# simochen/flowtrack.pytorch

Measured on AMD Instinct MI355X. Metric: pose crops/sec (ResNet-50 + 3-deconv head, 256x192), higher is better.
Workload: dtype fp16; 1 GPU; ResNet-50 pose head fp16, batch 64 x 256x192 synthetic crops per GPU (BASELINE.json configs[1]); per_gpu_batch=64, resident_batches=4, parallelism=dp1: batch sharded, one process per GPU

## Files before the change

### flowtrack/pytorch_amd/build.py

```python
from __future__ import annotations

import hashlib
import os
import subprocess
import sys

HERE = os.path.dirname(os.path.abspath(__file__))
ROOT = os.path.dirname(os.path.dirname(HERE))
CSRC = os.path.join(HERE, "csrc")
INCLUDE = os.path.join(ROOT, "include")
LIB_PATH = os.path.join(HERE, "libflowtrack_hip.so")
STAMP_PATH = os.path.join(HERE, ".libflowtrack_hip.stamp")

SOURCES = ["conv_igemm.hip", "conv_igemm8.hip", "bottleneck.hip", "bottleneck_rstat.hip", "bottleneck_stream.hip", "bottleneck_cluster.hip", "conv_direct.hip", "conv_wstat.hip", "aux_ops.hip", "flow_ops.hip", "crop_ops.hip", "runtime.hip"]
HEADERS = [os.path.join(CSRC, "ft_common.h"), os.path.join(CSRC, "conv_common.h"), os.path.join(CSRC, "conv_wstat.h"), os.path.join(INCLUDE, "flowtrack_hip.h")]
EXPORTS = os.path.join(CSRC, "exports.map")
ARCH = "gfx950"
FLAGS = ["-O3", "-std=c++17", "-fPIC", "-Wall", "-Wno-unused-function"]


def _hipcc() -> str:
    for cand in (os.environ.get("HIPCC"), "/opt/rocm/bin/hipcc", "hipcc"):
        if cand and (os.path.isabs(cand) and os.path.exists(cand) or not os.path.isabs(cand)):
            return cand
    raise RuntimeError("hipcc not found")


def _fingerprint() -> str:
    h = hashlib.sha256()
    for path in [os.path.join(CSRC, s) for s in SOURCES] + HEADERS + [EXPORTS]:
        with open(path, "rb") as f:
            h.update(f.read())
    h.update(" ".join(FLAGS + [ARCH]).encode())
    return h.hexdigest()


def is_current() -> bool:
    if not (os.path.exists(LIB_PATH) and os.path.exists(STAMP_PATH)):
        return False
    try:
        with open(STAMP_PATH) as f:
            return f.read().strip() == _fingerprint()
    except OSError:
        return False


def build(force: bool = False, verbose: bool = True) -> str:
    if not force and is_current():
        return LIB_PATH
    hipcc = _hipcc()
    objdir = os.path.join(HERE, "build")
    os.makedirs(objdir, exist_ok=True)
    procs = []
    objs = []
    fingerprint = _fingerprint()
    for src in SOURCES:
        obj = os.path.join(objdir, src.replace(".hip", ".o"))
        objs.append(obj)
        h = hashlib.sha256()
        for path in [os.path.join(CSRC, src)] + HEADERS:
            with open(path, "rb") as f:
                h.update(f.read())
        h.update(" ".join(FLAGS + [ARCH]).encode())
        want, stamp = h.hexdigest(), obj + ".stamp"
        if not force and os.path.exists(obj) and os.path.exists(stamp) and open(stamp).read().strip() == want:
            continue
        cmd = [hipcc, f"--offload-arch={ARCH}", *FLAGS, f"-I{INCLUDE}", f"-I{CSRC}", "-c",
               os.path.join(CSRC, src), "-o", obj]
        if verbose:
            print("[build]", " ".join(cmd), flush=True)
        procs.append((src, subprocess.Popen(cmd), stamp, want))
    for src, p, stamp, want in procs:
        if p.wait() != 0:
            raise RuntimeError(f"hipcc failed on {src}")
        with open(stamp, "w") as f:
            f.write(want)
    cmd = [hipcc, f"--offload-arch={ARCH}", "-shared", "-fPIC", f"-Wl,--version-script={EXPORTS}", *objs, "-o", LIB_PATH]
    if verbose:
        print("[build]", " ".join(cmd), flush=True)
    subprocess.check_call(cmd)
    with open(STAMP_PATH, "w") as f:
        f.write(fingerprint)
    return LIB_PATH


if __name__ == "__main__":
    build(force="--force" in sys.argv)
    print(LIB_PATH)
```

### flowtrack/pytorch_amd/csrc/conv_direct.hip

```cpp
#include <stdlib.h>

#include <type_traits>

#include "ft_common.h"
#include "conv_wstat.h"

namespace ft {
namespace {

struct CdParams {
  const char* x;
  const char* x2;
  const char* res;
  char* y;
  const char* ws;
  const float* scale;
  const float* shift;
  int M;
  int nc1, nc2;
  int x_cstride, x_coff;
  int HqWq, Wq;
  int x2_hi, x2_wi, x2_cstride, x2_coff, x2_stride;
  int y_cstride, y_coff, res_cstride, res_coff;
  int Cout, act;
// ... 1415 lines not shown
  if ((long long)d->N * d->Hi * d->Wi * d->x_cstride * 2 >= lim || M * d->y_cstride * 2 >= lim || (d->has_residual && M * d->res_cstride * 2 >= lim) ||
      (d->x2_cin && (long long)d->N * d->x2_hi * d->x2_wi * d->x2_cstride * 2 >= lim)) return FT_ERR_UNSUPPORTED;
  static const int cs_mode = dev_env_int("FT_CD_STATIONARY", 1);
  const bool cs256 = d->Cin == 256 && d->Cout % 128 == 0 && M > 65536, cs512 = cs_mode == 2 && d->Cin == 512 && d->Cout == 256 && M >= 32768;
  if (!taps && cs_mode != 0 && !d->x2_cin && !d->has_residual && (cs256 || cs512)) {
    const int bp = cs256 ? 128 : 64;
    *out = CdPlan{0, d->Cin / 64, 0, (int)((M + bp - 1) / bp), cs256 ? d->Cout / 128 : 1};
    return FT_OK;
  }
  if (!taps && M > 65536) return FT_ERR_UNSUPPORTED;
  const int npt = (int)((M + 95) / 96);
  const bool a_ok = d->Cout % 256 == 0 && d->Cin % 64 == 0 && d->x2_cin % 64 == 0;
  const bool b_ok = d->Cin % 256 == 0 && d->x2_cin % 256 == 0;
  if (!a_ok && !b_ok) return FT_ERR_UNSUPPORTED;
  int ks = a_ok ? 1 : 4;
  if (a_ok && b_ok && (long long)npt * (d->Cout / 256) < 160 && d->Cout <= 512) ks = 4;
  const int ck = ks == 1 ? 64 : 256;
  *out = CdPlan{ks, d->kh * d->kw * (d->Cin / ck), d->x2_cin / ck, npt, d->Cout / (ks == 1 ? 256 : 64)};
  return FT_OK;
}

template <int KSPLIT, bool HAS_RES, int NCH, bool TAPS = false>
static int cd_launch(const CdParams& p, hipStream_t s) {
  auto k = conv_direct_kernel<KSPLIT, HAS_RES, NCH, TAPS>;
  constexpr int lds = CdGeom<KSPLIT>::LDS_BYTES;
  static_assert(lds <= 163840, "LDS map");
  static bool attr_done[64] = {};
  int dev = 0;
  FT_HIP_CHECK(hipGetDevice(&dev));
  if (dev < 0 || dev >= 64 || !attr_done[dev]) {
    FT_HIP_CHECK(hipFuncSetAttribute(reinterpret_cast<const void*>(k), hipFuncAttributeMaxDynamicSharedMemorySize, lds));
    if (dev >= 0 && dev < 64) attr_done[dev] = true;
  }
  hipLaunchKernelGGL(k, dim3(p.npt * p.ncb), dim3(256), lds, s, p);
  FT_LAUNCH_CHECK("conv_direct_kernel");
  return FT_OK;
}

template <int KSPLIT>
static int cd_dispatch_taps(const CdParams& p, hipStream_t s) {
  if (KSPLIT == 1) {
    switch (p.nc1) {
      case 36: return cd_launch<KSPLIT, false, 36, true>(p, s);
      case 72: return cd_launch<KSPLIT, false, 72, true>(p, s);
      default: return cd_launch<KSPLIT, false, 0, true>(p, s);
    }
  }
  switch (p.nc1) {
    case 9: return cd_launch<KSPLIT, false, 9, true>(p, s);
    case 18: return cd_launch<KSPLIT, false, 18, true>(p, s);
    default: return cd_launch<KSPLIT, false, 0, true>(p, s);
  }
}

template <int KSPLIT, bool HAS_RES>
static int cd_dispatch(const CdParams& p, hipStream_t s) {
  const int n = p.nc1 + p.nc2;
  if (KSPLIT == 1) {
    switch (n) {
      case 4: return cd_launch<KSPLIT, HAS_RES, 4>(p, s);
      case 6: return cd_launch<KSPLIT, HAS_RES, 6>(p, s);
      case 8: return cd_launch<KSPLIT, HAS_RES, 8>(p, s);
      case 12: return cd_launch<KSPLIT, HAS_RES, 12>(p, s);
      case 16: return cd_launch<KSPLIT, HAS_RES, 16>(p, s);
      case 24: return cd_launch<KSPLIT, HAS_RES, 24>(p, s);
      default: return cd_launch<KSPLIT, HAS_RES, 0>(p, s);
    }
  }
  switch (n) {
    case 2: return cd_launch<KSPLIT, HAS_RES, 2>(p, s);
    case 4: return cd_launch<KSPLIT, HAS_RES, 4>(p, s);
    case 8: return cd_launch<KSPLIT, HAS_RES, 8>(p, s);
    default: return cd_launch<KSPLIT, HAS_RES, 0>(p, s);
  }
}

}
}

extern "C" int ft_conv_direct_supported(const ft_conv_desc* d) {
  ft::CdPlan pl;
  ft::C3Plan p3;
  ft::WsPlan pw;
  if (d && d->kh == 5) return ft::ws_plan(d, &pw);
  if (d && d->kh == 3 && ft::c3_plan(d, &p3) == FT_OK) return FT_OK;
  return ft::cd_plan(d, &pl);
}

extern "C" int ft_conv_direct_stream_id(const ft_conv_desc* d) {
  ft::CdPlan pl;
  ft::C3Plan p3;
  ft::WsPlan pw;
  if (d && d->kh == 5) return ft::ws_plan(d, &pw) == FT_OK ? (0x50000000 | pw.ncg) : -1;
  if (d && d->kh == 3 && ft::c3_plan(d, &p3) == FT_OK) return 0x40000000 | (p3.stride == 2 ? (p3.ipw == 2 ? 0x30000000 : 0x10000000) : 0) | (p3.ncb << 8) | p3.spt;
  if (ft::cd_plan(d, &pl) != FT_OK) return -1;
  return ((pl.ksplit + 1) << 24) | ((pl.nc1 + pl.nc2) << 12) | pl.ncb;
}

extern "C" long long ft_conv_direct_weight_bytes(const ft_conv_desc* d) {
  ft::CdPlan pl;
  ft::C3Plan p3;
  ft::WsPlan pw;
  if (d && d->kh == 5) return ft::ws_plan(d, &pw) == FT_OK ? ft::ws_weight_bytes(pw) : 0;
  if (d && d->kh == 3 && ft::c3_plan(d, &p3) == FT_OK) return (long long)p3.ncb * 4 * 9 * p3.spt * 8192;
  if (ft::cd_plan(d, &pl) != FT_OK) return 0;
  if (pl.ksplit == 0) return (long long)d->Cout * d->Cin * 2;
  return (long long)pl.ncb * (pl.nc1 + pl.nc2) * 32768;
}

extern "C" int ft_conv_direct_pack(const ft_conv_desc* d, const void* w_packed, int kpad, int cout_pad, void* wstream, ft_stream_t stream) {
  using namespace ft;
  C3Plan p3;
  if (d && d->kh == 5) {
    WsPlan pw;
    const int st = ws_plan(d, &pw);
    return st != FT_OK ? st : ws_pack(d, pw, w_packed, kpad, cout_pad, wstream, as_stream(stream));
  }
  if (d && d->kh == 3 && c3_plan(d, &p3) == FT_OK) {
    if (!w_packed || !wstream || kpad < 9 * d->Cin || cout_pad < d->Cout) return FT_ERR_INVALID_ARG;
    const int total = p3.ncb * 4 * 9 * p3.spt * 512;
    const dim3 pg(ceil_div(total, 256));
    const half_t* wsrc = static_cast<const half_t*>(w_packed);
    uint4_t* wdst = static_cast<uint4_t*>(wstream);
    if (p3.stride == 2 && p3.ipw == 2) hipLaunchKernelGGL(c3s2p_pack_kernel, pg, dim3(256), 0, as_stream(stream), wsrc, wdst, p3.ncb, kpad, cout_pad);
    else if (p3.stride == 2) hipLaunchKernelGGL(c3s2_pack_kernel<2>, pg, dim3(256), 0, as_stream(stream), wsrc, wdst, p3.ncb, kpad, cout_pad);
    else if (p3.spt == 4) hipLaunchKernelGGL(c3_pack_kernel<4>, pg, dim3(256), 0, as_stream(stream), wsrc, wdst, p3.ncb, kpad, cout_pad);
    else hipLaunchKernelGGL(c3_pack_kernel<2>, pg, dim3(256), 0, as_stream(stream), wsrc, wdst, p3.ncb, kpad, cout_pad);
    FT_LAUNCH_CHECK("c3_pack_kernel");
    return FT_OK;
  }
  CdPlan pl;
  const int st = cd_plan(d, &pl);
  if (st != FT_OK) return st;
  if (!w_packed || !wstream || kpad < d->kh * d->kw * d->Cin + d->x2_cin || cout_pad < d->Cout) return FT_ERR_INVALID_ARG;
  const int nchunk = pl.nc1 + pl.nc2;
  const int total = pl.ncb * nchunk * 2048;
  hipStream_t s = as_stream(stream);
  if (pl.ksplit == 0) {
    const int ntile = d->Cout / 32, ns = d->Cin / 16;
    hipLaunchKernelGGL(cs_pack_kernel, dim3(ceil_div(ntile * ns * 64, 256)), dim3(256), 0, s, static_cast<const half_t*>(w_packed),
                       static_cast<uint4_t*>(wstream), ntile, ns, kpad, cout_pad);
    FT_LAUNCH_CHECK("cs_pack_kernel");
    return FT_OK;
  }
  if (pl.ksplit == 1)
    hipLaunchKernelGGL(cd_pack_kernel<1>, dim3(ceil_div(total, 256)), dim3(256), 0, s, static_cast<const half_t*>(w_packed),
                       static_cast<uint4_t*>(wstream), nchunk, pl.ncb, kpad, cout_pad);
  else
    hipLaunchKernelGGL(cd_pack_kernel<4>, dim3(ceil_div(total, 256)), dim3(256), 0, s, static_cast<const half_t*>(w_packed),
                       static_cast<uint4_t*>(wstream), nchunk, pl.ncb, kpad, cout_pad);
  FT_LAUNCH_CHECK("cd_pack_kernel");
  return FT_OK;
}

extern "C" int ft_conv_direct_fwd(const ft_conv_desc* d, const void* x, const void* wstream, const float* scale, const float* shift,
                                  const void* residual, void* y, ft_stream_t stream) {
  using namespace ft;
  C3Plan p3;
  if (d && d->kh == 5) {
    WsPlan pw;
    const int st = ws_plan(d, &pw);
    return st != FT_OK ? st : ws_launch(d, pw, x, wstream, scale, shift, y, as_stream(stream));
  }
  if (d && d->kh == 3 && c3_plan(d, &p3) == FT_OK) {
    if (!x || !wstream || !y) return FT_ERR_INVALID_ARG;
    C3Params q{};
    q.x = static_cast<const char*>(x);
    q.y = static_cast<char*>(y);
    q.ws = static_cast<const char*>(wstream);
    q.scale = scale;
    q.shift = shift;
    q.HW = d->Hi * d->Wi; q.W = d->Wi; q.H = d->Hi; q.ipw = p3.ipw;
    q.Ho = p3.stride == 2 ? d->Ho : 0; q.Wo = p3.stride == 2 ? d->Wo : 0;
    q.strip_rows = p3.strip_rows; q.nstrips = p3.nstrips;
    q.M = p3.stride == 2 ? d->N * d->Ho * d->Wo : d->N * q.HW;
    q.x_cstride = d->x_cstride; q.x_coff = d->x_coff; q.y_cstride = d->y_cstride; q.y_coff = d->y_coff;
    q.Cout = d->Cout; q.act = d->act; q.slope = d->slope;
    q.npt = p3.npt; q.ncb = p3.ncb;
    q.x_bytes = (unsigned)((size_t)d->N * q.HW * d->x_cstride * 2);
    q.y_bytes = (unsigned)((size_t)q.M * d->y_cstride * 2);
    q.ws_bytes = (unsigned)ft_conv_direct_weight_bytes(d);
    q.wmajor = cd_wmajor((long long)d->N * q.HW * d->Cin * 2, q.ws_bytes, q.npt, q.ncb);
    if (p3.stride == 2 && p3.ipw == 2) {
      const int nld = (2 * q.HW * 256 + 4095) / 4096;
      if (p3.mt <= 2) return nld <= 16 ? c3s2p_launch<2, 16>(q, as_stream(stream)) : c3s2p_launch<2, 32>(q, as_stream(stream));
      return nld <= 24 ? c3s2p_launch<3, 24>(q, as_stream(stream)) : c3s2p_launch<3, 32>(q, as_stream(stream));
    }
    if (p3.stride == 2) return p3.mt == 1 ? c3s2_launch<1, 2>(q, as_stream(stream)) : c3s2_launch<2, 2>(q, as_stream(stream));
    if (p3.strip_rows) return c3_launch<3, 2, 4>(q, as_stream(stream));
    if (p3.spt == 4) return c3_launch<2, 4>(q, as_stream(stream));
    return p3.mt == 3 ? c3_launch<3, 2>(q, as_stream(stream)) : c3_launch<4, 2>(q, as_stream(stream));
  }
  CdPlan pl;
  const int st = cd_plan(d, &pl);
  if (st != FT_OK) return st;
  if (!x || !wstream || !y || ((d->has_residual || d->x2_cin) && !residual)) return FT_ERR_INVALID_ARG;
  if (pl.ksplit == 0) {
    CsParams q{};
    q.x = static_cast<const char*>(x);
    q.y = static_cast<char*>(y);
    q.ws = static_cast<const char*>(wstream);
    q.scale = scale;
    q.shift = shift;
    q.M = d->N * d->Ho * d->Wo;
    q.ntiles = pl.npt;
    q.x_cstride = d->x_cstride; q.x_coff = d->x_coff; q.y_cstride = d->y_cstride; q.y_coff = d->y_coff;
    q.Cout = d->Cout; q.act = d->act; q.slope = d->slope;
    q.x_bytes = (unsigned)((size_t)q.M * d->x_cstride * 2);
    q.y_bytes = (unsigned)((size_t)q.M * d->y_cstride * 2);
    q.ws_bytes = (unsigned)ft_conv_direct_weight_bytes(d);
    constexpr int lds = 2 * 65536;
    int gx = 256 / pl.ncb;
    gx = gx < 1 ? 1 : (gx > pl.npt ? pl.npt : gx);
    if (d->Cin == 256) {
      auto k = conv1x1_stream_kernel<16, 2, 2, 2, 2>;
      FT_RAISE_LDS(k, lds);
      hipLaunchKernelGGL(k, dim3(gx, pl.ncb), dim3(256), lds, as_stream(stream), q);
    } else {
      auto k = conv1x1_stream_kernel<32, 8, 1, 1, 2>;
      FT_RAISE_LDS(k, lds);
      hipLaunchKernelGGL(k, dim3(gx, 1), dim3(512), lds, as_stream(stream), q);
    }
    FT_LAUNCH_CHECK("conv1x1_stream_kernel");
    return FT_OK;
  }
  CdParams p{};
  p.x = static_cast<const char*>(x);
  p.y = static_cast<char*>(y);
  p.ws = static_cast<const char*>(wstream);
  p.scale = scale;
  p.shift = shift;
  p.M = d->N * d->Ho * d->Wo;
  p.nc1 = pl.nc1; p.nc2 = pl.nc2; p.npt = pl.npt; p.ncb = pl.ncb;
  p.x_cstride = d->x_cstride; p.x_coff = d->x_coff;
  p.HqWq = d->Ho * d->Wo; p.Wq = d->Wo;
  p.y_cstride = d->y_cstride; p.y_coff = d->y_coff;
  p.Cout = d->Cout; p.act = d->act; p.slope = d->slope;
  p.x_bytes = (unsigned)((size_t)d->N * d->Hi * d->Wi * d->x_cstride * 2);
  p.y_bytes = (unsigned)((size_t)p.M * d->y_cstride * 2);
  p.ws_bytes = (unsigned)ft_conv_direct_weight_bytes(d);
  const bool taps = d->kh != 1;
  p.cpt = d->Cin / (pl.ksplit == 1 ? 64 : 256); p.kw = d->kw; p.Hi = d->Hi; p.Wi = d->Wi; p.stride = d->stride; p.pad = d->pad;
  if (d->x2_cin) {
    p.x2 = static_cast<const char*>(residual);
    p.x2_hi = d->x2_hi; p.x2_wi = d->x2_wi; p.x2_cstride = d->x2_cstride; p.x2_coff = d->x2_coff; p.x2_stride = d->x2_stride;
    p.x2_bytes = (unsigned)((size_t)d->N * d->x2_hi * d->x2_wi * d->x2_cstride * 2);
// ... 16 lines not shown
```

### flowtrack/pytorch_amd/csrc/conv_wstat.h

```cpp
#pragma once
#include "ft_common.h"

namespace ft {

struct WsPlan {
  int ncg;
  int tiles_x, tiles_y;
  int npatches;
};

int ws_plan(const ft_conv_desc* d, WsPlan* out);
long long ws_weight_bytes(const WsPlan& pl);
int ws_pack(const ft_conv_desc* d, const WsPlan& pl, const void* w_packed, int kpad, int cout_pad, void* wstream, hipStream_t stream);
int ws_launch(const ft_conv_desc* d, const WsPlan& pl, const void* x, const void* wstream, const float* scale, const float* shift,
              void* y, hipStream_t stream);

}
```

### flowtrack/pytorch_amd/hip_ops.py

```python
from __future__ import annotations

import ctypes
import functools
import json
import os
import sys
from dataclasses import dataclass
from typing import List, Optional, Sequence, Tuple

import torch

from . import _lib
from ._lib import (FT_ACT_LEAKY, FT_ACT_NONE, FT_ACT_RELU, FT_LAYOUT_NCHW_F32, FT_LAYOUT_NHWC,
                   ConvDesc, ConvGeometry, FlowtrackHipError, check)

ACT_CODES = {None: FT_ACT_NONE, "none": FT_ACT_NONE, "relu": FT_ACT_RELU, "leaky": FT_ACT_LEAKY}


def require_gpu(device: torch.device) -> None:
    if device.type != "cuda" or not torch.cuda.is_available():
        raise FlowtrackHipError(
            "the flowtrack HIP path needs a ROCm GPU (model.cuda()); there is no CPU fallback — "
            "use oracle/ for CPU reference results")

# ... 669 lines not shown
        d.Cout, d.kh, d.kw = self.cout, self.k, self.k
        d.stride, d.pad, d.transposed = self.stride, self.pad, int(self.transposed)
        d.Ho, d.Wo = Ho, Wo
        out_c = self.tail_cout or self.cout
        if pool:
            if Ho % 2 or Wo % 2 or not isinstance(y, ActView) or residual is not None or self.tail_cout:
                raise FlowtrackHipError(f"{self.label}: the fused max-pool needs an even conv output and a plain NHWC result")
            d.pool = 1
        yH, yW = (Ho // 2, Wo // 2) if pool else (Ho, Wo)
        if isinstance(y, ActView):
            if (y.N, y.H, y.W) != (x.N, yH, yW) or y.C != out_c or y.t.dtype != self.dtype:
                raise FlowtrackHipError(f"{self.label}: output view mismatch {tuple(y.t.shape)} C={y.C}")
            d.y_cstride, d.y_coff, d.out_layout = y.cstride, y.coff, FT_LAYOUT_NHWC
            yt = y.t
        else:
            if tuple(y.shape) != (x.N, out_c, Ho, Wo) or y.dtype != torch.float32 or not y.is_contiguous():
                raise FlowtrackHipError(f"{self.label}: NCHW output must be contiguous fp32 {(x.N, out_c, Ho, Wo)}")
            d.y_cstride, d.y_coff, d.out_layout = 0, 0, FT_LAYOUT_NCHW_F32
            yt = y
        res_ptr = None
        if residual is not None:
            if (residual.N, residual.H, residual.W) != (x.N, Ho, Wo) or residual.C != self.cout:
                raise FlowtrackHipError(f"{self.label}: residual view mismatch")
            d.has_residual, d.res_cstride, d.res_coff = 1, residual.cstride, residual.coff
            res_ptr = residual.t.data_ptr()
        d.act, d.slope = self.act, self.slope
        if self.tail_cout:
            if residual is not None:
                raise FlowtrackHipError(f"{self.label}: a fused tail excludes a residual input")
            d.tail_cout = self.tail_cout
            res_ptr = self._tail.data_ptr()
        x_ptr, x_keep = x.t.data_ptr() if x_nchw is None else x_nchw.data_ptr(), x.t if x_nchw is None else x_nchw
        if x_nchw is not None:
            d.x_nchw_f32 = 1
        w, _, scale, shift = self._packed_for(d)
        if shift_n is not None:
            d.shift_nstride = self.cout
            if self.lib.ft_conv_shift_nstride_supported(ctypes.byref(d)) != 0:
                raise FlowtrackHipError(f"{self.label}: per-sample shift is not supported for this layer / shape")
            shift = shift_n(scale, shift)
            if tuple(shift.shape) != (x.N, self.cout) or shift.dtype != torch.float32 or not shift.is_contiguous():
                raise FlowtrackHipError(f"{self.label}: per-sample shift must be contiguous fp32 {(x.N, self.cout)}")
        flops = float(self.lib.ft_conv_flops(ctypes.byref(d)))
        ws = _direct_stream(self, d, w, x.t.device) if (self.k in (1, 3, 5) and isinstance(y, ActView) and not self.tail_cout and not pool) else None
        if ws is not None:
            dd = ConvDesc.from_buffer_copy(d)
            prog.begin_choice("conv|" + _desc_key(d))
            prog.option("direct")
            prog.flops += flops
            prog.conv_records.append((self.label, len(prog.calls), flops, dd))
            prog.add("ft_conv_direct_fwd", ctypes.byref(dd), x.t.data_ptr(), ws.data_ptr(),
                     scale.data_ptr() if scale is not None else None, shift.data_ptr() if shift is not None else None, res_ptr,
                     yt.data_ptr(), keep=(dd, x.t, yt, ws, scale, shift, residual.t if residual is not None else None))
            prog.option("igemm")
        self._record_igemm(prog, d, x, w, scale, shift, res_ptr, yt, residual, flops, x_ptr, x_keep)
        if ws is not None:
            prog.end_choice()

    def _record_igemm(self, prog: Program, d: ConvDesc, x: ActView, w, scale, shift, res_ptr, yt, residual, flops: float,
                      x_ptr=None, x_keep=None) -> None:
        x_ptr = x.t.data_ptr() if x_ptr is None else x_ptr
        x_keep = x.t if x_keep is None else x_keep
        prog.flops += flops
        prog.conv_records.append((self.label, len(prog.calls), flops, d))
        if prog._side:
            prog.add("ft_conv2d_fwd", ctypes.byref(d), x_ptr, w.data_ptr(),
                     scale.data_ptr() if scale is not None else None,
                     shift.data_ptr() if shift is not None else None, res_ptr, yt.data_ptr(),
                     keep=(d, x_keep, yt, w, scale, shift, residual.t if residual is not None else None, self._tail))
            return
        prog.need_workspace(self.lib.ft_conv_workspace_bytes(ctypes.byref(d)))
        prog.add("ft_conv2d_fwd_ws", ctypes.byref(d), x_ptr, w.data_ptr(),
                 scale.data_ptr() if scale is not None else None,
                 shift.data_ptr() if shift is not None else None, res_ptr, yt.data_ptr(), prog._ws_ptr, prog._ws_size,
                 keep=(d, x_keep, yt, w, scale, shift, residual.t if residual is not None else None, self._tail))


CONV_DIRECT = os.environ.get("FT_CONV_DIRECT", "1") != "0"
CONV_DIRECT_MAX_PIXELS = int(os.environ.get("FT_CONV_DIRECT_MAX_PIXELS", "65536"))


def _direct_stream(owner, d: ConvDesc, w: torch.Tensor, device) -> Optional[torch.Tensor]:
    lib = _lib.load()
    wstat = d.kh == 5 and d.Cin == 64 and d.stride == 2 and not d.x2_cin
    if not CONV_DIRECT or d.dtype != _lib.FT_F16 or (d.Cin + d.x2_cin < 256 and not wstat) or (d.kh == 5 and not wstat):
        return None
    if not wstat and d.N * d.Ho * d.Wo > CONV_DIRECT_MAX_PIXELS and not (CONV_DIRECT_MAX_PIXELS >= 65536 and d.kh == 1 and d.Cin in (256, 512)
                                                          and not d.x2_cin and not d.has_residual):
        return None
    if lib.ft_conv_direct_supported(ctypes.byref(d)) != 0:
        return None
    sid = int(lib.ft_conv_direct_stream_id(ctypes.byref(d)))
    if sid < 0:
        return None
    key = ("direct", sid, w.data_ptr())
    hit = owner._packed.get(key)
    if hit is None:
        ws = torch.empty(int(lib.ft_conv_direct_weight_bytes(ctypes.byref(d))), dtype=torch.uint8, device=device)
        check(lib.ft_conv_direct_pack(ctypes.byref(d), w.data_ptr(), int(w.shape[-1]), int(w.shape[-2]), ws.data_ptr(),
                                      current_stream_handle(device)), "ft_conv_direct_pack")
        torch.cuda.current_stream(device).synchronize()
        hit = owner._packed[key] = ws
    return hit


class FusedShortcutConv:

    def __init__(self, w3: torch.Tensor, bn3: dict, wd: torch.Tensor, bnd: dict, stride_d: int, *, dtype: torch.dtype,
                 device: torch.device, act: Optional[str] = "relu", label: str = ""):
        require_gpu(device)
        self.lib = _lib.load()
        self.dtype, self.device, self.code = dtype, device, _lib.dtype_code(dtype)
        self.cout, self.cin = w3.shape[0], w3.shape[1]
        self.cin2, self.stride_d = wd.shape[1], stride_d
        if wd.shape[0] != self.cout or w3.shape[2:] != (1, 1) or wd.shape[2:] != (1, 1):
            raise FlowtrackHipError(f"{label}: conv3 / downsample must be 1x1 convs with the same output channels")
        self.act, self.label = ACT_CODES[act], label

        def folded(w, bn):
            s, sh = fold_scale_shift(self.cout, self.cout, None, bn, torch.device("cpu"))
            return w.detach().to(torch.float32).cpu()[:, :, 0, 0] * s[:, None], sh
        self._w3, sh3 = folded(w3, bn3)
        self._wd, shd = folded(wd, bnd)
        self._shift = sh3 + shd
        self._packed = {}

    def _packed_for(self, d: ConvDesc):
        g = conv_geometry(d)
        key = g.key()
        hit = self._packed.get(key)
        if hit is None:
            w = torch.zeros((1, g.cout_pad, g.kpad), dtype=torch.float32)
            w[0, :self.cout, :self.cin] = self._w3
            w[0, :self.cout, g.cin_pad:g.cin_pad + self.cin2] = self._wd
            shift = torch.zeros(g.cout_pad, dtype=torch.float32)
            shift[:self.cout] = self._shift
            hit = self._packed[key] = (w.to(device=self.device, dtype=self.dtype).contiguous(), shift.to(self.device))
        return hit

    def record(self, prog: "Program", t2: ActView, x: ActView, y: ActView) -> None:
        if t2.C != self.cin or x.C != self.cin2 or y.C != self.cout:
            raise FlowtrackHipError(f"{self.label}: channel mismatch")
        if (x.N, (x.H - 1) // self.stride_d + 1, (x.W - 1) // self.stride_d + 1) != (t2.N, t2.H, t2.W) or (y.N, y.H, y.W) != (t2.N, t2.H, t2.W):
            raise FlowtrackHipError(f"{self.label}: shortcut / main / output sizes do not line up")
        d = ConvDesc()
        d.dtype = self.code
        d.N, d.Hi, d.Wi = t2.N, t2.H, t2.W
        d.Cin, d.x_cstride, d.x_coff = self.cin, t2.cstride, t2.coff
        d.Cout, d.kh, d.kw, d.stride, d.pad, d.transposed = self.cout, 1, 1, 1, 0, 0
        d.Ho, d.Wo = t2.H, t2.W
        d.y_cstride, d.y_coff, d.out_layout = y.cstride, y.coff, FT_LAYOUT_NHWC
        d.act, d.slope = self.act, 0.0
        d.x2_cin, d.x2_hi, d.x2_wi, d.x2_cstride, d.x2_coff, d.x2_stride = self.cin2, x.H, x.W, x.cstride, x.coff, self.stride_d
        w, shift = self._packed_for(d)
        flops = float(self.lib.ft_conv_flops(ctypes.byref(d)))
        ws = _direct_stream(self, d, w, t2.t.device)
        if ws is not None:
            dd = ConvDesc.from_buffer_copy(d)
            prog.begin_choice("conv|" + _desc_key(d))
            prog.option("direct")
            prog.flops += flops
            prog.conv_records.append((self.label, len(prog.calls), flops, dd))
            prog.add("ft_conv_direct_fwd", ctypes.byref(dd), t2.t.data_ptr(), ws.data_ptr(), None, shift.data_ptr(), x.t.data_ptr(),
                     y.t.data_ptr(), keep=(dd, t2.t, x.t, y.t, ws, shift))
            prog.option("igemm")
        prog.flops += flops
        prog.conv_records.append((self.label, len(prog.calls), flops, d))
# ... 446 lines not shown
```

Measured before the change: 58970 crops/s.

## Add weight-stationary kernel for 3x3 stride-2 128->128 convolution

Adds a new weight-stationary kernel for the layer2 first-block 3x3 stride-2 conv with 128 channels in and out. Each wave keeps its slice of weights in registers and streams 9x17 input patches into double-buffered LDS via buffer_load_lds. A persistent 256-workgroup grid runs the work, split across two waves that exchange partial sums through LDS. Previously this conv went through igemm, since Cin+x2_cin < 256 excluded it from the direct path. The goal is to cut redundant weight traffic and global load overhead, at the cost of a fixed grid and 512-thread blocks limited to one block per CU.

```diff
diff --git a/flowtrack/pytorch_amd/build.py b/flowtrack/pytorch_amd/build.py
--- a/flowtrack/pytorch_amd/build.py
+++ b/flowtrack/pytorch_amd/build.py
@@ -12,7 +12,7 @@
 LIB_PATH = os.path.join(HERE, "libflowtrack_hip.so")
 STAMP_PATH = os.path.join(HERE, ".libflowtrack_hip.stamp")
 
-SOURCES = ["conv_igemm.hip", "conv_igemm8.hip", "bottleneck.hip", "bottleneck_rstat.hip", "bottleneck_stream.hip", "bottleneck_cluster.hip", "conv_direct.hip", "conv_wstat.hip", "aux_ops.hip", "flow_ops.hip", "crop_ops.hip", "runtime.hip"]
+SOURCES = ["conv_igemm.hip", "conv_igemm8.hip", "bottleneck.hip", "bottleneck_rstat.hip", "bottleneck_stream.hip", "bottleneck_cluster.hip", "conv_direct.hip", "conv_wstat.hip", "conv_wstat3.hip", "aux_ops.hip", "flow_ops.hip", "crop_ops.hip", "runtime.hip"]
 HEADERS = [os.path.join(CSRC, "ft_common.h"), os.path.join(CSRC, "conv_common.h"), os.path.join(CSRC, "conv_wstat.h"), os.path.join(INCLUDE, "flowtrack_hip.h")]
 EXPORTS = os.path.join(CSRC, "exports.map")
 ARCH = "gfx950"
diff --git a/flowtrack/pytorch_amd/csrc/conv_direct.hip b/flowtrack/pytorch_amd/csrc/conv_direct.hip
--- a/flowtrack/pytorch_amd/csrc/conv_direct.hip
+++ b/flowtrack/pytorch_amd/csrc/conv_direct.hip
@@ -1521,7 +1521,9 @@
   ft::CdPlan pl;
   ft::C3Plan p3;
   ft::WsPlan pw;
+  ft::Ws3Plan pw3;
   if (d && d->kh == 5) return ft::ws_plan(d, &pw);
+  if (d && d->kh == 3 && ft::ws3_plan(d, &pw3) == FT_OK) return FT_OK;
   if (d && d->kh == 3 && ft::c3_plan(d, &p3) == FT_OK) return FT_OK;
   return ft::cd_plan(d, &pl);
 }
@@ -1530,7 +1532,9 @@
   ft::CdPlan pl;
   ft::C3Plan p3;
   ft::WsPlan pw;
+  ft::Ws3Plan pw3;
   if (d && d->kh == 5) return ft::ws_plan(d, &pw) == FT_OK ? (0x50000000 | pw.ncg) : -1;
+  if (d && d->kh == 3 && ft::ws3_plan(d, &pw3) == FT_OK) return 0x60000000;
   if (d && d->kh == 3 && ft::c3_plan(d, &p3) == FT_OK) return 0x40000000 | (p3.stride == 2 ? (p3.ipw == 2 ? 0x30000000 : 0x10000000) : 0) | (p3.ncb << 8) | p3.spt;
   if (ft::cd_plan(d, &pl) != FT_OK) return -1;
   return ((pl.ksplit + 1) << 24) | ((pl.nc1 + pl.nc2) << 12) | pl.ncb;
@@ -1540,7 +1544,9 @@
   ft::CdPlan pl;
   ft::C3Plan p3;
   ft::WsPlan pw;
+  ft::Ws3Plan pw3;
   if (d && d->kh == 5) return ft::ws_plan(d, &pw) == FT_OK ? ft::ws_weight_bytes(pw) : 0;
+  if (d && d->kh == 3 && ft::ws3_plan(d, &pw3) == FT_OK) return ft::ws3_weight_bytes();
   if (d && d->kh == 3 && ft::c3_plan(d, &p3) == FT_OK) return (long long)p3.ncb * 4 * 9 * p3.spt * 8192;
   if (ft::cd_plan(d, &pl) != FT_OK) return 0;
   if (pl.ksplit == 0) return (long long)d->Cout * d->Cin * 2;
@@ -1555,6 +1561,8 @@
     const int st = ws_plan(d, &pw);
     return st != FT_OK ? st : ws_pack(d, pw, w_packed, kpad, cout_pad, wstream, as_stream(stream));
   }
+  Ws3Plan pw3;
+  if (d && d->kh == 3 && ws3_plan(d, &pw3) == FT_OK) return ws3_pack(d, w_packed, kpad, cout_pad, wstream, as_stream(stream));
   if (d && d->kh == 3 && c3_plan(d, &p3) == FT_OK) {
     if (!w_packed || !wstream || kpad < 9 * d->Cin || cout_pad < d->Cout) return FT_ERR_INVALID_ARG;
     const int total = p3.ncb * 4 * 9 * p3.spt * 512;
@@ -1601,6 +1609,8 @@
     const int st = ws_plan(d, &pw);
     return st != FT_OK ? st : ws_launch(d, pw, x, wstream, scale, shift, y, as_stream(stream));
   }
+  Ws3Plan pw3;
+  if (d && d->kh == 3 && ws3_plan(d, &pw3) == FT_OK) return ws3_launch(d, pw3, x, wstream, scale, shift, y, as_stream(stream));
   if (d && d->kh == 3 && c3_plan(d, &p3) == FT_OK) {
     if (!x || !wstream || !y) return FT_ERR_INVALID_ARG;
     C3Params q{};
diff --git a/flowtrack/pytorch_amd/csrc/conv_wstat.h b/flowtrack/pytorch_amd/csrc/conv_wstat.h
--- a/flowtrack/pytorch_amd/csrc/conv_wstat.h
+++ b/flowtrack/pytorch_amd/csrc/conv_wstat.h
@@ -15,4 +15,15 @@
 int ws_launch(const ft_conv_desc* d, const WsPlan& pl, const void* x, const void* wstream, const float* scale, const float* shift,
               void* y, hipStream_t stream);
 
+struct Ws3Plan {
+  int tiles_x, tiles_y;
+  int npatches;
+};
+
+int ws3_plan(const ft_conv_desc* d, Ws3Plan* out);
+long long ws3_weight_bytes();
+int ws3_pack(const ft_conv_desc* d, const void* w_packed, int kpad, int cout_pad, void* wstream, hipStream_t stream);
+int ws3_launch(const ft_conv_desc* d, const Ws3Plan& pl, const void* x, const void* wstream, const float* scale, const float* shift,
+               void* y, hipStream_t stream);
+
 }
diff --git a/flowtrack/pytorch_amd/csrc/conv_wstat3.hip b/flowtrack/pytorch_amd/csrc/conv_wstat3.hip
--- /dev/null
+++ b/flowtrack/pytorch_amd/csrc/conv_wstat3.hip
@@ -0,0 +1,307 @@
+#include "conv_wstat.h"
+
+#include <stdlib.h>
+
+#include "conv_common.h"
+
+namespace ft {
+
+constexpr int kW3PR = 9, kW3PC = 17;
+constexpr int kW3Pieces = 40;
+constexpr int kW3PatchB = kW3Pieces * 1024;
+static_assert(kW3PR * kW3PC * 256 <= kW3PatchB && kW3Pieces % 8 == 0, "patch buffer");
+constexpr int kW3ExB = 8 * 2 * 1024;
+constexpr int kW3Lds = 2 * kW3PatchB + 2 * kW3ExB;
+constexpr int kW3NJ = 36;
+constexpr int kW3Grid = 256;
+
+__host__ __device__ constexpr int ws3_sigma(int r) { return 16 * ((r >> 2) & 1) + 4 * (r >> 3) + (r & 3); }
+
+struct Ws3Params {
+  const char* x;
+  char* y;
+  const char* ws;
+  const float* scale;
+  const float* shift;
+  int H, W, Ho, Wo;
+  int x_cstride, x_coff, y_cstride, y_coff;
+  int act;
+  float slope;
+  int tiles_x, tiles_y, npatches, ppw;
+  unsigned x_bytes, y_bytes, ws_bytes;
+  int dbg;
+};
+
+constexpr int kW3Ahead = 4;
+template <int H, int HS>
+__device__ __forceinline__ void ws3_read(unsigned abase, const int (&hk)[2][2], uint4_t& b) {
+  constexpr int tap = HS >> 2, c16 = HS & 3, ty = tap / 3, tx = tap % 3;
+  constexpr int toff = (ty * kW3PC + tx) * 256;
+  constexpr int lc = ((H << 3) | (c16 << 1)) << 4;
+  const unsigned a = abase + (unsigned)(lc ^ hk[tx >> 1][ty >> 1]);
+  asm volatile("ds_read_b128 %0, %1 offset:%2" : "=v"(b) : "v"(a), "n"(toff));
+}
+__device__ __forceinline__ void ws3_ex_rd(unsigned addr, float4_t (&fr)[2]) {
+  asm volatile("ds_read_b128 %0, %1" : "=v"(fr[0]) : "v"(addr));
+  asm volatile("ds_read_b128 %0, %1 offset:1024" : "=v"(fr[1]) : "v"(addr));
+}
+template <int NEWER>
+__device__ __forceinline__ void ws3_ex_sum(float4_t (&fr)[2], float (&v)[8]) {
+  asm volatile("s_waitcnt lgkmcnt(%2)" : "+v"(fr[0]), "+v"(fr[1]) : "n"(NEWER));
+#pragma unroll
+  for (int e = 0; e < 8; ++e) v[e] = v[e] + fr[e >> 2][e & 3];
+}
+__device__ __forceinline__ void ws3_ex_wr(unsigned addr, float4_t u0, float4_t u1) {
+  asm volatile("ds_write_b128 %0, %1" ::"v"(addr), "v"(u0) : "memory");
+  asm volatile("ds_write_b128 %0, %1 offset:1024" ::"v"(addr), "v"(u1) : "memory");
+}
+
+template <int H, typename Hook>
+__device__ __forceinline__ void ws3_mfma(const uint4_t (&wt)[kW3NJ], unsigned abase, const int (&hk)[2][2], float16_t& acc, Hook&& hook) {
+  uint4_t b[kW3Ahead + 1];
+  static_for<kW3Ahead>([&](auto hc) { ws3_read<H, decltype(hc)::value>(abase, hk, b[decltype(hc)::value]); });
+  static_for<kW3NJ>([&](auto hc) {
+    constexpr int hs = decltype(hc)::value;
+    if constexpr (hs + kW3Ahead < kW3NJ) ws3_read<H, hs + kW3Ahead>(abase, hk, b[(hs + kW3Ahead) % (kW3Ahead + 1)]);
+    constexpr int sl = hs % (kW3Ahead + 1);
+    constexpr int behind = kW3NJ - 1 - hs < kW3Ahead ? kW3NJ - 1 - hs : kW3Ahead;
+    asm volatile("s_waitcnt lgkmcnt(%1)" : "+v"(b[sl]) : "n"(behind));
+    acc = __builtin_amdgcn_mfma_f32_32x32x16_f16(__builtin_bit_cast(half8_t, wt[hs]), __builtin_bit_cast(half8_t, b[sl]), acc, 0, 0, 0);
+    hook(hc);
+  });
+}
+
+__global__ __launch_bounds__(512, 1) void conv3x3s2_wstat_kernel(const Ws3Params p) {
+#if defined(__HIP_DEVICE_COMPILE__)
+  extern __shared__ __attribute__((aligned(16))) char smem[];
+  typedef __attribute__((address_space(3))) void* lds_ptr;
+  const int tid = threadIdx.x, lane = tid & 63;
+  const int wave = __builtin_amdgcn_readfirstlane(tid >> 6);
+  const int c = wave & 3, h = wave >> 2;
+  const int l31 = lane & 31, lhi = lane >> 5;
+  const int wg = (blockIdx.x & 7) * (kW3Grid / 8) + (blockIdx.x >> 3);
+  const int p0 = wg * p.ppw;
+  const int p1 = p0 + p.ppw < p.npatches ? p0 + p.ppw : p.npatches;
+  if (p0 >= p1) return;
+  const __amdgpu_buffer_rsrc_t rsrc_x = __builtin_amdgcn_make_buffer_rsrc(const_cast<char*>(p.x), 0, p.x_bytes, 0x00020000);
+  const __amdgpu_buffer_rsrc_t rsrc_y = __builtin_amdgcn_make_buffer_rsrc(p.y, 0, p.y_bytes, 0x00020000);
+  const __amdgpu_buffer_rsrc_t rsrc_w = __builtin_amdgcn_make_buffer_rsrc(const_cast<char*>(p.ws), 0, p.ws_bytes, 0x00020000);
+  constexpr unsigned kOOB = 0x80000000u;
+
+  constexpr int NLD = kW3Pieces / 8;
+  const int l_pr0 = wave * 4 + (lane >> 4);
+  const int tiles = p.tiles_x * p.tiles_y;
+  int nx_iy0 = 0, nx_ix0 = 0, nx_origin = 0, nx_buf = 0;
+  bool nx_live = false;
+  auto nx_set = [&](int id, int bufi) {
+    nx_live = id < p1 && !(p.dbg & 2);
+    const int img = id / tiles, rem = id - img * tiles;
+    const int ty = rem / p.tiles_x, tx = rem - ty * p.tiles_x;
+    nx_iy0 = ty * 8 - 1, nx_ix0 = tx * 16 - 1;
+    nx_origin = ((img * p.H + nx_iy0) * p.W + nx_ix0) * p.x_cstride * 2;
+    nx_buf = bufi * kW3PatchB;
+  };
+  auto issue_one = [&](auto tc) {
+    constexpr int t = decltype(tc)::value;
+    int pr = l_pr0 + 32 * t;
+    asm volatile("" : "+v"(pr));
+    const int row = (pr * 241) >> 12, col = pr - row * kW3PC;
+    const int chunk = (lane & 15) ^ (((col >> 1) & 3) | (((row >> 1) & 3) << 2));
+    const int rel = ((row * p.W + col) * p.x_cstride + p.x_coff) * 2 + chunk * 16;
+    const bool ok = nx_live && row < kW3PR && (unsigned)(nx_iy0 + row) < (unsigned)p.H && (unsigned)(nx_ix0 + col) < (unsigned)p.W;
+    __builtin_amdgcn_raw_ptr_buffer_load_lds(rsrc_x, (lds_ptr)(smem + nx_buf + (t * 8 + wave) * 1024), 16,
+                                             ok ? (unsigned)(nx_origin + rel) : kOOB, 0, 0, 0);
+  };
+  nx_set(p0, 0);
+  static_for<NLD>([&](auto tc) { issue_one(tc); });
+
+  uint4_t wt[kW3NJ];
+  {
+    const int wbase = ((c * 2 + h) * kW3NJ) * 1024;
+#pragma unroll
+    for (int j = 0; j < kW3NJ; ++j) wt[j] = __builtin_amdgcn_raw_buffer_load_b128(rsrc_w, (unsigned)lane * 16u, wbase + j * 1024, 0);
+  }
+  const int e_ch = c * 32 + 16 * lhi + 8 * h;
+  float sc[8], sh[8];
+#pragma unroll
+  for (int e = 0; e < 8; ++e) {
+    sc[e] = p.scale ? p.scale[e_ch + e] : 1.f;
+    sh[e] = p.shift ? p.shift[e_ch + e] : 0.f;
+  }
+  const float act_k = p.act == FT_ACT_RELU ? 0.f : (p.act == FT_ACT_LEAKY ? p.slope : 1.f);
+
+  const int oy_l = l31 >> 3, ox_l = l31 & 7;
+  const int b_base = (2 * oy_l * kW3PC + 2 * ox_l) * 256;
+  int hk[2][2];
+#pragma unroll
+  for (int a2 = 0; a2 < 2; ++a2)
+#pragma unroll
+    for (int b2 = 0; b2 < 2; ++b2) hk[a2][b2] = (lhi ^ (((ox_l + a2) & 3) | (((oy_l + b2) & 3) << 2))) << 4;
+  const unsigned lds0 = (unsigned)(uintptr_t)(lds_ptr)smem;
+  const unsigned ex0 = lds0 + 2u * kW3PatchB;
+  const unsigned ex_rd_addr = ex0 + (unsigned)(wave * 2048 + lane * 16);
+  const unsigned ex_wr_addr = ex0 + (unsigned)((wave ^ 4) * 2048 + lane * 16);
+
+  float v[8];
+  float4_t fr[2];
+#pragma unroll
+  for (int e = 0; e < 8; ++e) v[e] = 0.f;
+  unsigned vo_prev = kOOB;
+  auto fin_c = [&]() {
+    half8_t o;
+#pragma unroll
+    for (int e = 0; e < 8; ++e) {
+      const float u = v[e] * sc[e] + sh[e];
+      o[e] = (half_t)act_mul(u, act_k);
+    }
+    __builtin_amdgcn_raw_buffer_store_b128(__builtin_bit_cast(uint4_t, o), rsrc_y, vo_prev, 0, 0);
+  };
+
+  asm volatile("s_waitcnt vmcnt(0)" ::: "memory");
+#pragma unroll
+  for (int j = 0; j < kW3NJ; ++j) asm volatile("" : "+v"(wt[j]));
+#pragma unroll
+  for (int e = 0; e < 8; ++e) asm volatile("" : "+v"(sc[e]), "+v"(sh[e]));
+  int k = 0;
+  unsigned long long tph[4] = {0, 0, 0, 0}, tprev = 0;
+#define WS3_TS(i) do { if (p.dbg & 32) { const unsigned long long t_ = __builtin_amdgcn_s_memtime(); tph[i] += t_ - tprev; tprev = t_; } } while (0)
+  if (p.dbg & 32) tprev = __builtin_amdgcn_s_memtime();
+  const unsigned long long tstart = tprev;
+  for (int id = p0; id < p1; ++id, ++k) {
+    const int bufi = k & 1;
+    if (k == 0) asm volatile("s_waitcnt vmcnt(0)" ::: "memory");
+    else asm volatile("s_waitcnt vmcnt(1)" ::: "memory");
+    WS3_TS(0);
+    asm volatile("s_waitcnt lgkmcnt(0)\n\ts_barrier" ::: "memory");
+    WS3_TS(1);
+    nx_set(id + 1, bufi ^ 1);
+    float16_t acc;
+#pragma unroll
+    for (int r = 0; r < 16; ++r) acc[r] = 0.f;
+    const unsigned abase = lds0 + (unsigned)(bufi * kW3PatchB + b_base);
+#pragma unroll
+    for (int a2 = 0; a2 < 2; ++a2)
+#pragma unroll
+      for (int b2 = 0; b2 < 2; ++b2) asm volatile("" : "+v"(hk[a2][b2]));
+    const unsigned ex_prev = (unsigned)((bufi ^ 1) * kW3ExB);
+    unsigned vo_next = kOOB;
+    auto hook = [&](auto hc) {
+      constexpr int hs = decltype(hc)::value;
+      if constexpr (hs < 2 * NLD && hs % 2 == 0) issue_one(std::integral_constant<int, hs / 2>{});
+      if constexpr (hs == 1) ws3_ex_rd(ex_rd_addr + ex_prev, fr);
+      if constexpr (hs == 3) ws3_ex_sum<2>(fr, v);
+      if constexpr (hs == 13) fin_c();
+      if constexpr (hs == 30) {
+        const int img = id / tiles, rem = id - img * tiles;
+        const int ty = rem / p.tiles_x, tx = rem - ty * p.tiles_x;
+        const int oy = ty * 4 + oy_l, ox = tx * 8 + ox_l;
+        vo_next = (oy < p.Ho && ox < p.Wo && !(p.dbg & 4))
+                      ? (unsigned)((((img * p.Ho + oy) * p.Wo + ox) * p.y_cstride + p.y_coff + e_ch) * 2) : kOOB;
+      }
+    };
+    if (h == 0) ws3_mfma<0>(wt, abase, hk, acc, hook);
+    else ws3_mfma<1>(wt, abase, hk, acc, hook);
+    WS3_TS(2);
+    asm volatile("s_nop 15\n\ts_nop 15" ::: "memory");
+    const unsigned ex_cur = ex_wr_addr + (unsigned)(bufi * kW3ExB);
+    if (h == 0) {
+      ws3_ex_wr(ex_cur, float4_t{acc[8], acc[9], acc[10], acc[11]}, float4_t{acc[12], acc[13], acc[14], acc[15]});
+#pragma unroll
+      for (int e = 0; e < 8; ++e) v[e] = acc[e];
+    } else {
+      ws3_ex_wr(ex_cur, float4_t{acc[0], acc[1], acc[2], acc[3]}, float4_t{acc[4], acc[5], acc[6], acc[7]});
+#pragma unroll
+      for (int e = 0; e < 8; ++e) v[e] = acc[8 + e];
+    }
+    vo_prev = vo_next;
+    WS3_TS(3);
+  }
+  if (p.dbg & 32) {
+    asm volatile("s_waitcnt vmcnt(0) lgkmcnt(0)\n\ts_barrier" ::: "memory");
+    if ((tid & 63) == 0 && p.y_bytes >= (unsigned)(kW3Grid * 8 * 64)) {
+      unsigned long long* o = reinterpret_cast<unsigned long long*>(p.y) + (blockIdx.x * 8 + wave) * 8;
+      for (int i = 0; i < 4; ++i) o[i] = tph[i];
+      o[4] = o[5] = 0;
+      o[6] = tprev - tstart;
+      o[7] = (unsigned long long)k;
+    }
+    return;
+  }
+  asm volatile("s_waitcnt lgkmcnt(0)\n\ts_barrier" ::: "memory");
+  ws3_ex_rd(ex_rd_addr + (unsigned)(((k - 1) & 1) * kW3ExB), fr);
+  ws3_ex_sum<0>(fr, v);
+  fin_c();
+  asm volatile("s_waitcnt vmcnt(0)" ::: "memory");
+#endif
+}
+
+__global__ __launch_bounds__(256) void ws3_pack_kernel(const half_t* __restrict__ w, uint4_t* __restrict__ out, int kpad, int cout_pad) {
+  const int idx = blockIdx.x * 256 + threadIdx.x;
+  if (idx >= 4 * 2 * kW3NJ * 64) return;
+  const int lane = idx & 63;
+  int f = idx >> 6;
+  const int j = f % kW3NJ; f /= kW3NJ;
+  const int h = f & 1, c = f >> 1;
+  const int co = c * 32 + ws3_sigma(lane & 31);
+  const int k = (j >> 2) * 128 + 64 * h + (j & 3) * 16 + 8 * (lane >> 5);
+  uint4_t v = {0u, 0u, 0u, 0u};
+  if (co < cout_pad && k + 8 <= kpad) v = *reinterpret_cast<const uint4_t*>(w + (size_t)co * kpad + k);
+  out[idx] = v;
+}
+
+int ws3_plan(const ft_conv_desc* d, Ws3Plan* out) {
+  if (!d || !out) return FT_ERR_INVALID_ARG;
+  if (d->act == FT_ACT_LEAKY && !(d->slope >= 0.f && d->slope <= 1.f)) return FT_ERR_UNSUPPORTED;
+  if (d->dtype != FT_F16 || d->transposed || d->kh != 3 || d->kw != 3 || d->stride != 2 || d->pad != 1 || d->Cin != 128 || d->Cout != 128) return FT_ERR_UNSUPPORTED;
+  if (d->x2_cin || d->has_residual || d->tail_cout || d->pool || d->x_wpitch || d->shift_nstride || d->x_nchw_f32 || d->out_layout != FT_LAYOUT_NHWC) return FT_ERR_UNSUPPORTED;
+  if (d->N <= 0 || d->Hi <= 0 || d->Wi <= 0 || d->Hi > 16384 || d->Wi > 16384) return FT_ERR_UNSUPPORTED;
+  if (d->Ho != (d->Hi + 2 - 3) / 2 + 1 || d->Wo != (d->Wi + 2 - 3) / 2 + 1 || d->Ho <= 0 || d->Wo <= 0) return FT_ERR_UNSUPPORTED;
+  if (d->x_coff % 8 || d->x_cstride % 8 || d->y_coff % 8 || d->y_cstride % 8) return FT_ERR_UNSUPPORTED;
+  if (d->x_cstride < d->x_coff + d->Cin || d->y_cstride < d->y_coff + d->Cout) return FT_ERR_UNSUPPORTED;
+  const long long lim = 1LL << 31;
+  if (((long long)d->N * d->Hi + 18) * (d->Wi + 18) * d->x_cstride * 2 >= lim || (long long)d->N * d->Ho * d->Wo * d->y_cstride * 2 >= lim) return FT_ERR_UNSUPPORTED;
+  out->tiles_x = ceil_div(d->Wo, 8);
+  out->tiles_y = ceil_div(d->Ho, 4);
+  const long long np = (long long)d->N * out->tiles_x * out->tiles_y;
+  if (np >= (1 << 24)) return FT_ERR_UNSUPPORTED;
+  out->npatches = (int)np;
+  return FT_OK;
+}
+
+long long ws3_weight_bytes() { return 4LL * 2 * kW3NJ * 1024; }
+
+int ws3_pack(const ft_conv_desc* d, const void* w_packed, int kpad, int cout_pad, void* wstream, hipStream_t stream) {
+  if (!w_packed || !wstream || kpad < 9 * 128 || cout_pad < d->Cout) return FT_ERR_INVALID_ARG;
+  const int total = 4 * 2 * kW3NJ * 64;
+  hipLaunchKernelGGL(ws3_pack_kernel, dim3(ceil_div(total, 256)), dim3(256), 0, stream, static_cast<const half_t*>(w_packed),
+                     static_cast<uint4_t*>(wstream), kpad, cout_pad);
+  FT_LAUNCH_CHECK("ws3_pack_kernel");
+  return FT_OK;
+}
+
+int ws3_launch(const ft_conv_desc* d, const Ws3Plan& pl, const void* x, const void* wstream, const float* scale, const float* shift,
+               void* y, hipStream_t stream) {
+  if (!x || !wstream || !y) return FT_ERR_INVALID_ARG;
+  static const int dbg = dev_env_int("FT_CD_DBG", 0);
+  Ws3Params q{};
+  q.x = static_cast<const char*>(x);
+  q.y = static_cast<char*>(y);
+  q.ws = static_cast<const char*>(wstream);
+  q.scale = scale;
+  q.shift = shift;
+  q.H = d->Hi; q.W = d->Wi; q.Ho = d->Ho; q.Wo = d->Wo;
+  q.x_cstride = d->x_cstride; q.x_coff = d->x_coff; q.y_cstride = d->y_cstride; q.y_coff = d->y_coff;
+  q.act = d->act; q.slope = d->slope;
+  q.tiles_x = pl.tiles_x; q.tiles_y = pl.tiles_y; q.npatches = pl.npatches;
+  q.ppw = ceil_div(pl.npatches, kW3Grid);
+  q.x_bytes = (unsigned)((size_t)d->N * d->Hi * d->Wi * d->x_cstride * 2);
+  q.y_bytes = (unsigned)((size_t)d->N * d->Ho * d->Wo * d->y_cstride * 2);
+  q.ws_bytes = (unsigned)ws3_weight_bytes();
+  q.dbg = dbg;
+  FT_RAISE_LDS(conv3x3s2_wstat_kernel, kW3Lds);
+  hipLaunchKernelGGL(conv3x3s2_wstat_kernel, dim3(kW3Grid), dim3(512), kW3Lds, stream, q);
+  FT_LAUNCH_CHECK("conv3x3s2_wstat_kernel");
+  return FT_OK;
+}
+
+}
diff --git a/flowtrack/pytorch_amd/hip_ops.py b/flowtrack/pytorch_amd/hip_ops.py
--- a/flowtrack/pytorch_amd/hip_ops.py
+++ b/flowtrack/pytorch_amd/hip_ops.py
@@ -775,7 +775,8 @@
 
 def _direct_stream(owner, d: ConvDesc, w: torch.Tensor, device) -> Optional[torch.Tensor]:
     lib = _lib.load()
-    wstat = d.kh == 5 and d.Cin == 64 and d.stride == 2 and not d.x2_cin
+    wstat = (d.kh == 5 and d.Cin == 64 and d.stride == 2 and not d.x2_cin) or \
+            (d.kh == 3 and d.stride == 2 and d.pad == 1 and d.Cin == 128 and d.Cout == 128 and not d.x2_cin and not d.has_residual)
     if not CONV_DIRECT or d.dtype != _lib.FT_F16 or (d.Cin + d.x2_cin < 256 and not wstat) or (d.kh == 5 and not wstat):
         return None
     if not wstat and d.N * d.Ho * d.Wo > CONV_DIRECT_MAX_PIXELS and not (CONV_DIRECT_MAX_PIXELS >= 65536 and d.kh == 1 and d.Cin in (256, 512)
```

Measured after the change: 59440 crops/s, median of 6. No clear change (+0.8%).
